# brown-ivl/manus

Hardware: AMD Instinct MI355X
Metric: train iters/sec (fwd+bwd) 300k Gaussians @1080p, 8 views; PSNR parity (higher is better)
Workload: dtype f32

## Files before the change

### manus_amd/csrc/raster_fwd.hip

```cpp
#include <atomic>
#include <mutex>

#include "instance_math.h"
#include "il_list.h"

#include <cstdlib>
#include <cstring>
#include <map>
#include <string>
#include <vector>

thread_local char g_mgr_err[512] = {0};

int g_mgr_prof_on = 0;
namespace {
struct ProfRec { const char* name; hipEvent_t a, b; };
std::vector<ProfRec> g_prof_recs;
std::vector<hipEvent_t> g_prof_pool;
hipEvent_t prof_event() {
    if (!g_prof_pool.empty()) { hipEvent_t e = g_prof_pool.back(); g_prof_pool.pop_back(); return e; }
    hipEvent_t e;
    if (hipEventCreate(&e) != hipSuccess) return nullptr;
    return e;
}
}

void mgr_prof_begin(const char* name, hipStream_t stream) {
    ProfRec r{name, prof_event(), prof_event()};
    if (r.a) (void)hipEventRecord(r.a, stream);
    g_prof_recs.push_back(r);
}
void mgr_prof_end(hipStream_t stream) {
    if (!g_prof_recs.empty() && g_prof_recs.back().b) (void)hipEventRecord(g_prof_recs.back().b, stream);
}

static std::string g_prof_filter;
static int g_prof_period = 1, g_prof_seen = 0;
bool mgr_prof_match(const char* name) {
    if (!(g_prof_filter.empty() || g_prof_filter == name)) return false;
    return g_prof_period <= 1 || (g_prof_seen++ % g_prof_period) == 0;
}
extern "C" int mgr_profile_sample_every(int n) {
    g_prof_period = n < 1 ? 1 : n;
    g_prof_seen = 0;
    return MGR_OK;
}

extern "C" int mgr_profile_enable(int on) {
    g_mgr_prof_on = on ? 1 : 0;
    return MGR_OK;
}

extern "C" int mgr_profile_filter(const char* kernel_name) {
    g_prof_filter = kernel_name ? kernel_name : "";
    return MGR_OK;
}

extern "C" int mgr_profile_report(char* buf, size_t len, void* stream_) {
    hipStream_t stream = (hipStream_t)stream_;
    MGR_HIP(hipStreamSynchronize(stream));
    std::map<std::string, std::pair<long, double>> agg;
    std::vector<std::string> order;
    for (auto& r : g_prof_recs) {
        float ms = 0.f;
        if (r.a && r.b && hipEventElapsedTime(&ms, r.a, r.b) == hipSuccess) {
            auto it = agg.find(r.name);
            if (it == agg.end()) { order.push_back(r.name); agg[r.name] = {1, ms}; }
            else { it->second.first += 1; it->second.second += ms; }
        }
        if (r.a) g_prof_pool.push_back(r.a);
        if (r.b) g_prof_pool.push_back(r.b);
    }
    g_prof_recs.clear();
    std::string out;
    for (auto& n : order) {
        char line[256];
        snprintf(line, sizeof(line), "%s %ld %.6f\n", n.c_str(), agg[n].first, agg[n].second);
        out += line;
    }
    if (buf && len) {
        size_t k = out.size() < len - 1 ? out.size() : len - 1;
        memcpy(buf, out.data(), k);
        buf[k] = 0;
    }
    return MGR_OK;
}

extern "C" int mgr_version(void) { return MGR_VERSION; }
int mgr_bwd_variant_bits(void);
extern "C" int mgr_raster_repair_max_tiles(void) { return MGR_REP_MAX_TILES; }

extern "C" int mgr_build_variant(void) {
    int bits = mgr_bwd_variant_bits();
#ifdef FWD_KO_DEEP
    bits |= 1;
#endif
#if defined(MGR_STATS) || defined(MGR_TIMELINE) || defined(FWD_PROF) || defined(BIN_PROF) || defined(DBS_PROF)
    bits |= 2;
#endif
#if defined(FWD_PF1) || defined(FWD_LDS_PIPE1)
    bits |= 4;
#endif
    if (MGR_BIN_BLOCK != 1024 || MGR_GREC_BYTES != 64 || MGR_DB_BUCKETS != 1024 || MGR_DB_ITEM != 768 || MGR_DB_RANK_MAX != 2048 ||
        MGR_DB_RANK_LARGE != 3072)
        bits |= 4;
    return bits;
}
extern "C" const char* mgr_last_error(void) { return g_mgr_err; }

extern "C" int mgr_raster_record_bytes(void) { return (int)sizeof(MgrGRec); }
extern "C" size_t mgr_raster_workspace_bytes(int V, int N, int W, int H, int64_t cap) {
    return mgr_layout(V, N, W, H, cap).total;
}

__device__ __forceinline__ uint32_t block_excl_scan(uint32_t val, uint32_t* s_wave ,
                                                    uint32_t& block_total) {
    const int lane = threadIdx.x & 63, wave = threadIdx.x >> 6, nw = blockDim.x >> 6;
    const uint32_t incl = mgr_wave_incl_scan_u32(val);
    if (lane == 63) s_wave[wave] = incl;
    __syncthreads();
    if (threadIdx.x == 0) {
        uint32_t run = 0;
        for (int w = 0; w < nw; ++w) {
            uint32_t t = s_wave[w];
            s_wave[w] = run;
            run += t;
        }
        s_wave[nw] = run;
    }
    __syncthreads();
    block_total = s_wave[nw];
    uint32_t r = s_wave[wave] + incl - val;
    __syncthreads();
    return r;
}

#ifndef MGR_FWD_GRID
#define MGR_FWD_GRID (256 * 24)
#endif
#ifndef PRE_THREADS
#define PRE_THREADS 512
#endif
#define EMIT_THREADS 1024

struct DbRange { float zmin, scale; };
__device__ __forceinline__ DbRange db_range_reduce(const uint32_t* __restrict__ slots , int nslots, uint32_t* s_zr ) {
    uint32_t lo_c = 0u, hi = 0u;
    for (int k = threadIdx.x; k < nslots; k += blockDim.x) { lo_c = max(lo_c, slots[2 * k]); hi = max(hi, slots[2 * k + 1]); }
    lo_c = mgr_wave_max_u32(lo_c); hi = mgr_wave_max_u32(hi);
    if ((threadIdx.x & 63) == 0 && hi) { atomicMax(&s_zr[0], lo_c); atomicMax(&s_zr[1], hi); }
    __syncthreads();
    lo_c = s_zr[0]; hi = s_zr[1];
    DbRange r;
    r.zmin = __uint_as_float(~lo_c);
    const float ext = __uint_as_float(hi) - r.zmin;
    r.scale = (hi != 0u && ext > 0.0f) ? (float)(MGR_DB_BUCKETS - 1) / ext : 0.0f;
    return r;
}
__device__ __forceinline__ uint32_t db_bucket(float z, const DbRange r) {
    const float f = (z - r.zmin) * r.scale;
    return f > 0.0f ? min((uint32_t)f, (uint32_t)MGR_DB_BUCKETS - 1u) : 0u;
}
__device__ __forceinline__ bool db_takes_part(int radius, ushort4 rc, unsigned long long am) {
    const uint32_t tiles = (uint32_t)((rc.z - rc.x) * (rc.w - rc.y));
    return radius > 0 && tiles > 0u && (tiles > 64u || am != 0ull);
}

__device__ __forceinline__ void pre_tail(int N, int gx, int gy, int v, int i, const ProjOut& po, float op_i,
                                         const float col[3], uint32_t* s_scan, uint32_t* s_hist, int lds_hist,
                                         MgrGRec* __restrict__ grec, float* __restrict__ depth,
                                         ushort4* __restrict__ rect, unsigned long long* __restrict__ alive,
                                         uint32_t* __restrict__ pair_off, uint32_t* __restrict__ tile_count,
                                         int32_t* __restrict__ radii, MgrHeader* hdr, uint32_t* __restrict__ zr_slot,
                                         const uint32_t* __restrict__ zcut_v = nullptr) {
    const int tid = threadIdx.x, T = gx * gy;
    const int radius = po.radius, x0 = po.x0, y0 = po.y0, x1 = po.x1, y1 = po.y1;
    const uint32_t tiles = (uint32_t)((x1 - x0) * (y1 - y0));
    {
        const uint32_t zb = (radius > 0 && tiles > 0u) ? __float_as_uint(po.zv) : 0u;
        const uint32_t wmax = mgr_wave_max_u32(zb), wminc = mgr_wave_max_u32(zb ? ~zb : 0u);
        if ((tid & 63) == 0 && wmax) { atomicMax(&s_scan[23], wmax); atomicMax(&s_scan[22], wminc); }
    }
    unsigned long long amask = ~0ull;
    if (radius > 0 && !(zcut_v && tiles <= 64)) {
        const bool small = tiles <= 64;
        const MgrCull cull = mgr_cull_init(po.px, po.py, po.ca, po.cb, po.cc, mgr_qmax(op_i));
        if (small) amask = 0ull;
        int k = 0;
// ... 1310 lines not shown
        const uint4 q = db_rec[(size_t)v * N + p];
        r.gid = db_order[(size_t)v * N + p];
        const uint32_t w = q.y & 0xFFFFu, h = q.y >> 16;
        r.xy = ((uint32_t)((int)(q.x & 0xFFFFu) - (int)box.x) & 0xFFFFu) | ((uint32_t)((int)(q.x >> 16) - (int)box.y) << 16);
        r.wh = q.y;
        r.tiles = w * h;
        r.alo = q.z; r.ahi = q.w;
    }
    return r;
}
__device__ __noinline__ BinRec bin_spread_lane(uint32_t j, const BinRec cur, const uint32_t* s_vend) {
    BinRec r = {0u, 0u, 0u, 0u, 0u, 0u};
    const bool on = j < s_vend[63];
    int lo = 0, hi = 63;
    while (lo < hi) {
        const int mid = (lo + hi) >> 1;
        if (s_vend[mid] > j) hi = mid; else lo = mid + 1;
    }
    BinRec q;
    q.xy = (uint32_t)__shfl((int)cur.xy, lo, 64); q.wh = (uint32_t)__shfl((int)cur.wh, lo, 64);
    q.alo = (uint32_t)__shfl((int)cur.alo, lo, 64); q.ahi = (uint32_t)__shfl((int)cur.ahi, lo, 64);
    q.gid = (uint32_t)__shfl((int)cur.gid, lo, 64); q.tiles = (uint32_t)__shfl((int)cur.tiles, lo, 64);
    if (!on) return r;
    if (q.tiles <= 64u) return q;
    const uint32_t piece = j - (lo ? s_vend[lo - 1] : 0u), qw = q.wh & 0xFFFFu, per_row = (qw + 63u) / 64u;
    const uint32_t row = piece / per_row, px = piece - row * per_row, ww = min(64u, qw - 64u * px);
    r.xy = ((uint32_t)(bin_x0(q.xy) + (int)(64u * px)) & 0xFFFFu) | ((uint32_t)(bin_y0(q.xy) + (int)row) << 16);
    r.wh = ww | (1u << 16);
    const unsigned long long ones = ww >= 64u ? ~0ull : ((1ull << ww) - 1ull);
    r.alo = (uint32_t)ones; r.ahi = (uint32_t)(ones >> 32);
    r.gid = q.gid;
    r.tiles = ww;
    return r;
}

__device__ __forceinline__ void bin_batch_by_instance(const BinRec& r, const BinRec* s_rec, uint32_t* s_cur, int bw, int lane,
                                                      uint32_t* __restrict__ sorted_gid, uint32_t cap) {
    const int g = lane >> 4, kq = lane & 15;
    const unsigned long long quad_ok = __ballot(r.tiles <= 16u);
    int i = 0;
#pragma unroll 1
    while (i < 64) {
        if ((i & 3) == 0 && ((quad_ok >> i) & 0xFull) == 0xFull) {
            const BinRec q = s_rec[i + g];
            const uint32_t w = q.wh & 0xFFFFu;
            const uint32_t ty = (uint32_t)(((float)kq + 0.5f) * __frcp_rn((float)max(w, 1u)));
            const uint32_t tx = kq - ty * w;
            const unsigned long long am = ((unsigned long long)q.ahi << 32) | q.alo;
            const bool valid = (uint32_t)kq < q.tiles && ((am >> kq) & 1ull);
            uint32_t* cur = &s_cur[valid ? (bin_y0(q.xy) + (int)ty) * bw + bin_x0(q.xy) + (int)tx : 0];
            uint32_t pa = 0, pb = 0, pc = 0, pd = 0;
            if (valid && g == 0) pa = atomicAdd(cur, 1u);
            __builtin_amdgcn_wave_barrier();
            if (valid && g == 1) pb = atomicAdd(cur, 1u);
            __builtin_amdgcn_wave_barrier();
            if (valid && g == 2) pc = atomicAdd(cur, 1u);
            __builtin_amdgcn_wave_barrier();
            if (valid && g == 3) pd = atomicAdd(cur, 1u);
            __builtin_amdgcn_wave_barrier();
            const uint32_t pos = pa | pb | pc | pd;
            if (valid && pos < cap) sorted_gid[pos] = q.gid;
            i += 4;
        } else {
            const BinRec q = s_rec[i];
            if (q.tiles) {
                const uint32_t w = q.wh & 0xFFFFu;
                const unsigned long long am = ((unsigned long long)q.ahi << 32) | q.alo;
                const bool small = q.tiles <= 64u;
                for (uint32_t k = (uint32_t)lane; k < q.tiles; k += 64) {
                    const uint32_t ty = k / w, tx = k - ty * w;
                    if (small && !((am >> k) & 1ull)) continue;
                    const uint32_t pos = atomicAdd(&s_cur[(bin_y0(q.xy) + (int)ty) * bw + bin_x0(q.xy) + (int)tx], 1u);
                    if (pos < cap) sorted_gid[pos] = q.gid;
                }
            }
            __builtin_amdgcn_wave_barrier();
            i += 1;
        }
    }
}

#define BIN_PAIR_CAP 1024
#ifdef BIN_PROF
__device__ unsigned long long g_binprof[8 * 4096];
#define BP(k) { const long long now_ = wall_clock64(); acc_[k] += now_ - tp_; tp_ = now_; }
#else
#define BP(k)
#endif
#define BIN_SC_THREADS 192
__constant__ unsigned long long c_row_comb[65] = {0x0000000000000000ull, 0x5555555555555555ull, 0x1111111111111111ull, 0x1041041041041041ull, 0x0101010101010101ull, 0x1004010040100401ull, 0x1001001001001001ull, 0x0100040010004001ull, 0x0001000100010001ull, 0x0040001000040001ull, 0x1000010000100001ull, 0x0000100000400001ull, 0x0001000001000001ull, 0x0010000004000001ull, 0x0100000010000001ull, 0x1000000040000001ull, 0x0000000100000001ull, 0x0000000400000001ull, 0x0000001000000001ull, 0x0000004000000001ull, 0x0000010000000001ull, 0x0000040000000001ull, 0x0000100000000001ull, 0x0000400000000001ull, 0x0001000000000001ull, 0x0004000000000001ull, 0x0010000000000001ull, 0x0040000000000001ull, 0x0100000000000001ull, 0x0400000000000001ull, 0x1000000000000001ull, 0x4000000000000001ull, 0x0000000000000001ull, 0x0000000000000001ull, 0x0000000000000001ull, 0x0000000000000001ull, 0x0000000000000001ull, 0x0000000000000001ull, 0x0000000000000001ull, 0x0000000000000001ull, 0x0000000000000001ull, 0x0000000000000001ull, 0x0000000000000001ull, 0x0000000000000001ull, 0x0000000000000001ull, 0x0000000000000001ull, 0x0000000000000001ull, 0x0000000000000001ull, 0x0000000000000001ull, 0x0000000000000001ull, 0x0000000000000001ull, 0x0000000000000001ull, 0x0000000000000001ull, 0x0000000000000001ull, 0x0000000000000001ull, 0x0000000000000001ull, 0x0000000000000001ull, 0x0000000000000001ull, 0x0000000000000001ull, 0x0000000000000001ull, 0x0000000000000001ull, 0x0000000000000001ull, 0x0000000000000001ull, 0x0000000000000001ull, 0x0000000000000001ull};
#define BIN_SC_FIXED_BYTES (2 * 64 * sizeof(BinRec) + 2 * BIN_PAIR_CAP * 4 + 3 * 64 * 4 + 16 + 66 * 8)
#define BIN_MID_TILES 1536
__device__ __forceinline__ bool bin_sc_mine(ushort4 box, int masks) {
    const uint32_t tb = (uint32_t)box.z * (uint32_t)box.w;
    if (tb == 0u) return false;
    const int tier = tb <= (uint32_t)BIN_MID_TILES ? BIN_MID_TILES : (tb <= (uint32_t)BIN_SMALL_TILES ? BIN_SMALL_TILES : 0);
    return tier == masks;
}
template <int MASKS, bool SPREAD>
__global__ __launch_bounds__(BIN_SC_THREADS) void k_bin_scatter(int N, int T, int nblk, int bb, const uint32_t* __restrict__ db_nvis,
                                                                const ushort4* __restrict__ db_bbox,
                                                                const uint32_t* __restrict__ db_order,
                                                                const uint4* __restrict__ db_rec,
                                                                const uint32_t* __restrict__ bin_mat,
                                                                uint32_t* __restrict__ sorted_gid, uint32_t cap,
                                                                MgrHeader* hdr, int skipped) {
    constexpr bool SMALL = MASKS > 0;
    extern __shared__ __attribute__((aligned(16))) uint32_t s_mem[];
    BinRec* s_rec = (BinRec*)s_mem;
    unsigned long long* s_mask = (unsigned long long*)(s_mem + 2 * 64 * (sizeof(BinRec) / 4));
    uint32_t* s_pairs = (uint32_t*)(s_mask + MASKS);
    uint32_t* s_gid = s_pairs + 2 * BIN_PAIR_CAP;
    uint32_t* s_info = s_gid + 2 * 64;
    unsigned long long* s_comb = (unsigned long long*)(s_info + 4);
    uint32_t* s_vend = (uint32_t*)(s_comb + 66);
    uint32_t* s_cur = s_vend + 64;
    const int v = blockIdx.y, b = blockIdx.x, tid = threadIdx.x, lane = tid & 63, wave = tid >> 6;
    const ushort4 box = db_bbox[v];
    if (!bin_sc_mine(box, MASKS)) {
        if (MASKS == BIN_MID_TILES && skipped && b == 0 && tid == 0) {
            const uint32_t tb = (uint32_t)box.z * (uint32_t)box.w;
            if ((tb > (uint32_t)BIN_SMALL_TILES && (skipped & MGR_SKIP_BOX_LARGE)) || (tb > (uint32_t)BIN_MID_TILES && tb <= (uint32_t)BIN_SMALL_TILES && (skipped & MGR_SKIP_BOX_MID)))
                atomicOr(&hdr->overflow, MGR_OVF_TIER);
        }
        return;
    }
    const uint32_t nvis = db_nvis[v], p0 = (uint32_t)b * (uint32_t)bb;
    if (p0 >= nvis) return;
    const uint32_t p1 = min(p0 + (uint32_t)bb, nvis);
    const int bw = box.z;
    const int nbatch = (int)((p1 - p0 + 63u) / 64u);
    BinRec nxt = {0u, 0u, 0u, 0u, 0u, 0u};
    if (wave == 0) nxt = bin_load(N, v, p0 + lane, nvis, box, db_order, db_rec);
    {
        const int TB = (int)box.z * (int)box.w;
        const uint32_t* row = bin_mat + ((size_t)v * nblk + b) * T;
        int k = tid;
        for (; k + 3 * BIN_SC_THREADS < TB; k += 4 * BIN_SC_THREADS) {
            const uint32_t a0 = row[k], a1 = row[k + BIN_SC_THREADS], a2 = row[k + 2 * BIN_SC_THREADS], a3 = row[k + 3 * BIN_SC_THREADS];
            s_cur[k] = a0; s_cur[k + BIN_SC_THREADS] = a1; s_cur[k + 2 * BIN_SC_THREADS] = a2; s_cur[k + 3 * BIN_SC_THREADS] = a3;
        }
        for (; k < TB; k += BIN_SC_THREADS) s_cur[k] = row[k];
        if (SMALL) for (k = tid; k < TB; k += BIN_SC_THREADS) s_mask[k] = 0ull;
        if (tid < 65) s_comb[tid] = c_row_comb[tid];
    }
    const unsigned long long lt = (1ull << lane) - 1ull;
#ifdef BIN_PROF
    long long acc_[6] = {0, 0, 0, 0, 0, 0};
    const long long t00_ = wall_clock64();
    long long tp_ = t00_;
#endif
    int src_it = 0;
    uint32_t v_total = 0, v_off = 0;
    bool v_mapped = false;
    BinRec cur = {0u, 0u, 0u, 0u, 0u, 0u};
    bool last_emitted = false;
    bool met_big = false;
#pragma unroll 1
    for (int it = 0; SPREAD || it <= nbatch; ++it) {
        __syncthreads();
        BP(5)
        if (wave == 0) {
            const int d = it & 1;
            if (SPREAD && last_emitted) break;
            if (SPREAD || it < nbatch) {
                BinRec r;
                if constexpr (!SPREAD) {
                    r = nxt;
                    BP(0)
                    if (it + 1 < nbatch) nxt = bin_load(N, v, p0 + 64u * (uint32_t)(it + 1) + lane, nvis, box, db_order, db_rec);
                } else {
                if (v_off >= v_total) {
                    cur = nxt;
                    BP(0)
                    ++src_it;
                    if (src_it < nbatch) nxt = bin_load(N, v, p0 + 64u * (uint32_t)src_it + lane, nvis, box, db_order, db_rec);
                    const uint32_t cw = cur.wh & 0xFFFFu, ch = cur.wh >> 16;
                    v_mapped = __ballot(cur.tiles > 64u) != 0ull;
                    v_off = 0u;
                    v_total = 64u;
                    if (v_mapped) {
                        met_big = true;
                        const uint32_t nl = cur.tiles == 0u ? 0u : (cur.tiles <= 64u ? 1u : ch * ((cw + 63u) / 64u));
                        const uint32_t ve = mgr_wave_incl_scan_u32(nl);
                        v_total = (uint32_t)__builtin_amdgcn_readlane((int)ve, 63);
                        s_vend[lane] = ve;
                        __builtin_amdgcn_wave_barrier();
                        if (v_total == 0u) v_total = 1u;
                    }
                }
                r = cur;
                if (v_mapped) r = bin_spread_lane(v_off + (uint32_t)lane, cur, s_vend);
                v_off += 64u;
                last_emitted = v_off >= v_total && src_it >= nbatch;
                }
                const unsigned long long am = ((unsigned long long)r.ahi << 32) | r.alo;
                const bool big = !SPREAD && r.tiles > 64u;
                const bool use = r.tiles != 0u && !big;
                const uint32_t w = r.wh & 0xFFFFu;
                unsigned long long amE = 0ull;
                if (use) {
                    const unsigned long long rb = w >= 64u ? ~0ull : ((1ull << w) - 1ull);
                    const unsigned long long evens = rb * s_comb[min(w, 64u)];
                    const unsigned long long rowm = (bin_y0(r.xy) & 1) ? (w >= 64u ? 0ull : evens << w) : evens;
                    amE = am & rowm;
                }
                const unsigned long long amU = use ? am : 0ull;
                const uint32_t cntE = (uint32_t)__popcll(amE), cntO = (uint32_t)__popcll(amU & ~amE);
                const uint32_t incl = mgr_wave_incl_scan_u32(cntE | (cntO << 16));
                const uint32_t P = (uint32_t)__builtin_amdgcn_readlane((int)incl, 63);
                const uint32_t PE = P & 0xFFFFu, PO = P >> 16;
                BP(1)
                const bool any_big = !SPREAD && __ballot(big) != 0ull;
                met_big = met_big || any_big;
                if (!any_big && PE + PO <= (uint32_t)BIN_PAIR_CAP) {
                    uint32_t* pl = s_pairs + d * BIN_PAIR_CAP;
                    uint32_t oE = (incl & 0xFFFFu) - cntE, oO = (incl >> 16) - cntO;
                    const float rw = __frcp_rn((float)max(w, 1u));
                    const int org = bin_y0(r.xy) * bw + bin_x0(r.xy);
                    unsigned long long m = amU;
                    while (m) {
                        const uint32_t k = (uint32_t)__builtin_ctzll(m);
                        m &= m - 1ull;
                        const uint32_t ty = (uint32_t)(((float)k + 0.5f) * rw), tx = k - ty * w;
                        const uint32_t isE = (uint32_t)((amE >> k) & 1ull);
                        const uint32_t at = isE ? oE : (uint32_t)BIN_PAIR_CAP - 1u - oO;
                        oE += isE;
                        oO += 1u - isE;
                        pl[at] = (uint32_t)(org + (int)ty * bw + (int)tx) | ((uint32_t)lane << 16);
                    }
                    s_gid[d * 64 + lane] = r.gid;
                    if (lane == 0) s_info[d] = P | (last_emitted ? 0x80000000u : 0u);
                } else {
                    s_rec[d * 64 + lane] = r;
                    if (lane == 0) s_info[d] = 0x7FFFFFFFu | (last_emitted ? 0x80000000u : 0u);
                }
                BP(2)
            }
        } else if (it >= 1) {
            const int d = (it - 1) & 1;
            const uint32_t Praw = s_info[d], Pboth = Praw & 0x7FFFFFFFu;
            if (Pboth != 0x7FFFFFFFu) {
                const bool odd = wave == 2;
                const uint32_t P = odd ? Pboth >> 16 : Pboth & 0xFFFFu;
                const uint32_t* const plist = s_pairs + d * BIN_PAIR_CAP;
                auto pl = [&](uint32_t i) -> uint32_t { return plist[odd ? (uint32_t)BIN_PAIR_CAP - 1u - i : i]; };
                const uint32_t* gl = s_gid + d * 64;
                uint32_t pr_n = lane < P ? pl((uint32_t)lane) : 0u;
                if (SMALL) {
                    uint32_t first_p = 0u, rank_p = 0u, gid_p = 0u, src_p = 0u;
                    bool valid_p = false;
#pragma unroll 1
                    for (uint32_t c = 0; c < P + 64; c += 64) {
                        const bool valid = c + lane < P;
                        const uint32_t pr = pr_n;
                        if (c + 64 < P) pr_n = (c + 64 + lane < P) ? pl(c + 64u + (uint32_t)lane) : 0u;
                        const uint32_t t = pr & 0xFFFFu;
                        if (valid) atomicOr(&s_mask[t], 1ull << lane);
                        __builtin_amdgcn_wave_barrier();
                        const unsigned long long mm = valid ? *(volatile unsigned long long*)&s_mask[t] : (1ull << lane);
                        const uint32_t rank = (uint32_t)__popcll(mm & lt);
                        const bool leader = valid && rank == 0u;
                        uint32_t first = 0u;
                        if (leader) {
                            first = atomicAdd(&s_cur[t], (uint32_t)__popcll(mm));
                            s_mask[t] = 0ull;
                        }
                        const uint32_t gid = gl[pr >> 16];
                        if (c > 0) {
                            const uint32_t f = (uint32_t)__shfl((int)first_p, (int)src_p, 64);
                            const uint32_t pos = f + rank_p;
                            if (valid_p && pos < cap) sorted_gid[pos] = gid_p;
                        }
                        first_p = first; rank_p = rank; gid_p = gid; valid_p = valid;
                        src_p = (uint32_t)__builtin_ctzll(mm);
                    }
                } else {
#pragma unroll 1
                    for (uint32_t c = 0; c < P; c += 64) {
                        const bool valid = c + lane < P;
                        const uint32_t pr = pr_n;
                        if (c + 64 < P) pr_n = (c + 64 + lane < P) ? pl(c + 64u + (uint32_t)lane) : 0u;
                        const uint32_t t = pr & 0xFFFFu;
                        uint32_t pos = 0u, cend = 1u;
                        if (valid) {
                            pos = atomicAdd(&s_cur[t], 1u);
                            cend = *(volatile uint32_t*)&s_cur[t];
                        }
                        const uint32_t gid = gl[pr >> 16];
                        unsigned long long todo = __ballot(valid && cend - pos > 1u);
                        while (todo) {
                            const int first = __builtin_ctzll(todo);
                            const uint32_t tstar = (uint32_t)__builtin_amdgcn_readlane((int)t, first);
                            const bool in = valid && t == tstar;
                            const unsigned long long grp = __ballot(in);
                            if (in) pos = cend - (uint32_t)__popcll(grp) + (uint32_t)__popcll(grp & lt);
                            todo &= ~grp;
                        }
                        if (valid && pos < cap) sorted_gid[pos] = gid;
                    }
                }
                BP(3)
            } else if (wave == 1) {
                const BinRec r = s_rec[d * 64 + lane];
                bin_batch_by_instance(r, s_rec + d * 64, s_cur, bw, lane, sorted_gid, cap);
                BP(4)
            }
            if (Praw & 0x80000000u) break;
        }
    }
    if (wave == 0 && lane == 0 && met_big && (*(volatile uint32_t*)&hdr->tiers & 4u) == 0u) atomicOr(&hdr->tiers, 4u);
#ifdef BIN_PROF
    {
        const int wid = blockIdx.y * gridDim.x + blockIdx.x;
        if (lane == 0 && wid < 4096) {
            if (wave == 0) { g_binprof[wid * 8 + 0] = acc_[0]; g_binprof[wid * 8 + 1] = acc_[1]; g_binprof[wid * 8 + 2] = acc_[2];
                             g_binprof[wid * 8 + 5] = (unsigned long long)(tp_ - t00_); g_binprof[wid * 8 + 6] = (unsigned long long)t00_;
                             g_binprof[wid * 8 + 7] = (unsigned long long)tp_; }
            else { g_binprof[wid * 8 + 3] = acc_[3]; g_binprof[wid * 8 + 4] = acc_[4]; }
        }
    }
#endif
}

struct FwdRec {
    float4 a, b;
    float c;
};

#ifdef MGR_STATS
__device__ unsigned long long g_fhist[5][65];
extern "C" int mgr_debug_fhist(unsigned long long* dst) {
    return (int)hipMemcpyFromSymbol(dst, HIP_SYMBOL(g_fhist), sizeof(unsigned long long) * 5 * 65);
}
#define FH(r, c, v) do { const int c_ = (c); const unsigned long long v_ = (unsigned long long)(v); if (lane == 0) atomicAdd(&g_fhist[r][c_], v_); } while (0)
#endif


#ifdef FWD_PROF
__device__ unsigned long long g_fprof[8];
extern "C" int mgr_debug_fprof(unsigned long long* dst) {
    return (int)hipMemcpyFromSymbol(dst, HIP_SYMBOL(g_fprof), sizeof(unsigned long long) * 8);
}
#ifndef FWD_PROF_MIN
#define FWD_PROF_MIN 0u
#endif
#ifndef FWD_PROF_MAX
#define FWD_PROF_MAX 0xFFFFFFFFu
#endif
#define FP(k) { const long long now_ = wall_clock64(); if (fp_on_) facc_[k] += now_ - ftp_; ftp_ = now_; }
#else
#define FP(k)
#endif
#ifndef FWD_WAVES_EU
#define FWD_WAVES_EU 4
#endif
#define FWD_OCC __attribute__((amdgpu_waves_per_eu(FWD_WAVES_EU, FWD_WAVES_EU)))
#ifdef MGR_TIMELINE
#define TLW_PER_WAVE 24
__device__ unsigned long long g_tlw[MGR_FWD_GRID * 4 * TLW_PER_WAVE * 4];
extern "C" int mgr_debug_timeline_w(void* dst, unsigned int* n) {
    *n = MGR_FWD_GRID * 4 * TLW_PER_WAVE;
    hipError_t e = hipMemcpyFromSymbol(dst, HIP_SYMBOL(g_tlw), sizeof(g_tlw));
    return (int)e;
}
#endif
__device__ __forceinline__ float mgr_sel(unsigned long long m, float a, float b) {
    float r;
    asm("v_cndmask_b32 %0, %1, %2, %3" : "=v"(r) : "v"(b), "v"(a), "s"(m));
    return r;
}
__device__ __forceinline__ uint32_t mgr_selu(unsigned long long m, uint32_t a, uint32_t b) {
    uint32_t r;
    asm("v_cndmask_b32 %0, %1, %2, %3" : "=v"(r) : "v"(b), "v"(a), "s"(m));
    return r;
}
__device__ __forceinline__ bool mgr_fwd_pair_step(const float4& R0, const float4& R1, const float4& R2, const float4& R3, const float4& R4,
                                                  const mgr_v2f fpx2, const mgr_v2f fpy2, float& Tr, mgr_v2f& C01, float& C2, uint32_t& last,
                                                  unsigned long long& done_m, const unsigned long long exec_m) {
    mgr_v2f al;
    unsigned long long ma, mb;
    mgr_pair_alpha_masks(R0, R1, R2, fpx2, fpy2, al, ma, mb);
    {
        const unsigned long long keep = ma & ~done_m;
        const float a = mgr_sel(keep, al.x, 0.0f);
        const float testT = Tr * (1.0f - a);
        const unsigned long long stop = __builtin_amdgcn_ballot_w64(testT < 0.0001f);
        const unsigned long long contrib = keep & ~stop;
        const float w = mgr_sel(contrib, a * Tr, 0.0f);
        C01 += mgr_v2f{R3.x, R3.y} * w;
        C2 += R4.x * w;
        Tr = mgr_sel(stop, Tr, testT);
        last = mgr_selu(contrib, __float_as_uint(R4.z), last);
        done_m |= stop;
    }
    {
        const unsigned long long keep = mb & ~done_m;
        const float a = mgr_sel(keep, al.y, 0.0f);
        const float testT = Tr * (1.0f - a);
        const unsigned long long stop = __builtin_amdgcn_ballot_w64(testT < 0.0001f);
        const unsigned long long contrib = keep & ~stop;
        const float w = mgr_sel(contrib, a * Tr, 0.0f);
// ... 1002 lines not shown
        MGR_HIP(side.init());
        MGR_HIP(hipEventRecord(side.fork, stream));
        MGR_HIP(hipStreamWaitEvent(side.stream, side.fork, 0));
        { MGR_PROF("k_tile_split", stream); hipLaunchKernelGGL(k_tile_split, dim3(256), dim3(SORT_THREADS), 0, stream,
                           tile_start, (const uint32_t*)(ws + L.tile_queue), (unsigned long long*)(ws + L.keys),
                           (unsigned long long*)(ws + L.keys2), (uint4*)(ws + L.groups),
                           (uint32_t*)(ws + L.sorted_gid), hdr, (uint32_t)cap); }
        { MGR_PROF("k_tile_sort_small", side.stream); hipLaunchKernelGGL(k_tile_sort_small, dim3(256 * 8), dim3(256), 0, side.stream,
                           tile_start, (const uint32_t*)(ws + L.tile_queue),
                           (const unsigned long long*)(ws + L.keys), (uint32_t*)(ws + L.sorted_gid), hdr,
                           (uint32_t)cap); }
        MGR_HIP(hipEventRecord(side.join, side.stream));
        { MGR_PROF("k_tile_sort", stream); hipLaunchKernelGGL(k_tile_sort, dim3(512), dim3(RS_THREADS), SORT_LDS_KEYS * 8 + RS_WAVES * 256 * 4 + 256, stream,
                           tile_start, (const uint32_t*)(ws + L.tile_queue),
                           (const unsigned long long*)(ws + L.keys), (const unsigned long long*)(ws + L.keys2),
                           (const uint4*)(ws + L.groups), (uint32_t*)(ws + L.sorted_gid), hdr, (uint32_t)cap); }
        MGR_HIP(hipStreamWaitEvent(stream, side.join, 0));
        MGR_LAUNCH_CHECK("k_tile_sort", stream, debug);
    }
    }
    if (!do_blend) return MGR_OK;
    { MGR_PROF("k_blend_fwd", stream); hipLaunchKernelGGL(k_blend_fwd, dim3(MGR_FWD_GRID), dim3(256), 0, stream, N, W, H, gx, gy, VT, bg,
                       (const uint32_t*)(ws + L.tile_queue), (const uint4*)(ws + L.tile_qrec), (const uint32_t*)(ws + L.sorted_gid), (const MgrGRec*)(ws + L.grec), out_color,
                       (uint32_t*)(ws + L.n_contrib), (uint32_t*)(ws + L.tile_done), (uint32_t*)(ws + L.tile_qdone),
                       (float4*)(ws + L.ckpt), hdr, (const uint32_t*)(ws + L.tile_zused), (uint32_t*)(ws + L.tile_qend), bg_filled ? 1 : 0); }
    if (repair && N > 0) {
        { MGR_PROF("k_repair_scan", stream);
          hipLaunchKernelGGL(k_repair_prep, dim3(V), dim3(256), 0, stream, T, gx, hdr, rep_all, (const uint32_t*)(ws + L.tile_zused),
                             (const uint32_t*)(ws + L.tile_zwin));
          hipLaunchKernelGGL(k_repair_scan, dim3(REP_SCAN_SEGS, V), dim3(REP_SCAN_THREADS), 0, stream, N, T, gx, hdr, rep_all, (const int32_t*)radii,
                             (const ushort4*)(ws + L.rect), (const float*)(ws + L.depth), (const MgrGRec*)(ws + L.grec)); }
        { MGR_PROF("k_repair_blend", stream);
          hipLaunchKernelGGL(k_repair_blend, dim3(128), dim3(RS_THREADS), REP_BLEND_LDS, stream, N, W, H, gx, T, hdr, rep_all, bg,
                             (uint32_t*)(ws + L.sorted_gid), (const MgrGRec*)(ws + L.grec), out_color, (uint32_t*)(ws + L.n_contrib),
                             (uint32_t*)(ws + L.tile_qdone), (float4*)(ws + L.ckpt)); }
        MGR_LAUNCH_CHECK("k_repair_blend", stream, debug);
    }
    IlListArgs ll = g_loss_list.take(workspace);
    if (ll.nbx) {
        if (ll.H != H || ll.W != W || ll.list_views != V) return mgr_fail(MGR_EINVAL, "attached loss list: views or image size differ from the forward's");
        ll.tile_start = tile_start;
    }
    const int n_item_blocks = (VT + 255) / 256;
    const MgrFeatStamp stamp = {{(uint32_t)V, (uint32_t)N, (uint32_t)W, (uint32_t)H, (uint32_t)cap}, use_cut ? MGR_FEAT_CUT : 0u};
    { MGR_PROF("k_fwd_items", stream); hipLaunchKernelGGL(k_fwd_items, dim3((unsigned)(n_item_blocks + ll.nbx * V)), dim3(256), 0, stream, (const uint4*)(ws + L.tile_qrec),
                       (const uint32_t*)(ws + L.tile_qdone), (uint32_t*)(ws + L.tile_done), (uint4*)(ws + L.items), hdr,
                       N, T, (const uint32_t*)(ws + L.sorted_gid), (const float*)(ws + L.depth), (const uint32_t*)(ws + L.tile_zused),
                       (const uint32_t*)(ws + L.tile_qend), (uint32_t*)(ws + L.tile_zcut), g_mirror.take(workspace),
                       g_cut_frac, (uint32_t)g_cut_min, g_cut_range, g_cut_rel, gx, g_cut_interior,
                       (const uint32_t*)(ws + L.tile_queue), VT, (unsigned char*)(ws + L.tile_bgok), (const float*)out_color, bg, rep_all,
                       (uint32_t)g_cut_penalty, (uint32_t*)(ws + L.tile_zwin), ll, n_item_blocks, stamp); }
    MGR_LAUNCH_CHECK("k_blend_fwd", stream, debug);
    return MGR_OK;
}

extern "C" int mgr_raster_forward(int V, int N, int W, int H, const float* cams, const float* bg,
                                  const float* means3D, int64_t s_means, const float* cov3D,
                                  int64_t s_cov, const float* colors, int64_t s_col,
                                  const float* opacity, int64_t s_op, float* out_color,
                                  int32_t* radii, void* workspace, size_t workspace_bytes,
                                  int64_t cap, int flags, void* stream_) {
    return raster_forward_impl(V, N, W, H, cams, bg, means3D, s_means, cov3D, s_cov, colors, s_col, opacity, s_op,
                               nullptr, out_color, radii, workspace, workspace_bytes, cap, flags, stream_);
}

extern "C" int mgr_views_forward(int V, int N, int B, int n_articulated, int sh_half, int W, int H, const float* cams, const float* bg,
                                 const float* xyz, const float* log_scale, const float* rot,
                                 const float* opacity_logit, const float* f_dc, const float* f_rest,
                                 const float* skin_w, const float* transforms, float* out_color,
                                 int32_t* radii, void* workspace, size_t workspace_bytes, int64_t cap,
                                 int flags, void* stream_) {
    if (N > 0 && (!xyz || !log_scale || !rot || !opacity_logit || !f_dc || !f_rest || (skin_w && !transforms)))
        return mgr_fail(MGR_EINVAL, "mgr_views_forward: null pointer");
    if (skin_w && (B <= 0 || B > MGR_MAX_BONES)) return mgr_fail(MGR_EINVAL, "mgr_views_forward: bad B");
    if (skin_w && (n_articulated < 0 || n_articulated > N)) return mgr_fail(MGR_EINVAL, "mgr_views_forward: bad n_articulated");
    if (sh_half && ((uintptr_t)f_rest & 15)) return mgr_fail(MGR_EINVAL, "mgr_views_forward: fp16 f_rest must be 16-byte aligned");
    const CanonInputs ci = {B, skin_w ? n_articulated : 0, sh_half ? 1 : 0, xyz, log_scale, rot, opacity_logit, f_dc, f_rest, skin_w, transforms};
    return raster_forward_impl(V, N, W, H, cams, bg, nullptr, 0, nullptr, 0, nullptr, 0, nullptr, 0, &ci, out_color,
                               radii, workspace, workspace_bytes, cap, flags, stream_);
}

#ifdef BIN_PROF
extern "C" int mgr_binprof(unsigned long long* out) {
    MGR_HIP(hipMemcpyFromSymbol(out, HIP_SYMBOL(g_binprof), 8 * 8 * 4096));
    return 0;
}
#endif
extern "C" int mgr_raster_layout(int V, int N, int W, int H, int64_t cap, size_t* out, int n_out) {
    const MgrLayout L = mgr_layout(V, N, W, H, cap);
    const size_t v[] = {L.header, L.grec, L.depth, L.rect, L.alive, L.pair_off, L.tile_count, L.tile_start,
                        L.tile_cursor, L.tile_done, L.tile_queue, L.chunk_start, L.items, L.ckpt, L.keys,
                        L.sorted_gid, L.final_T, L.n_contrib, L.pair_tag, L.pair_grad, L.total, L.inst_grad, L.inst_tag,
                        L.db_nvis, L.db_bbox, L.db_order, L.tile_zcut, L.tile_zused, L.tile_qend, L.tile_rep, L.rep_unit, L.rep_cnt, L.tile_zwin};
    const int n = (int)(sizeof(v) / sizeof(v[0]));
    for (int i = 0; i < n && i < n_out; ++i) out[i] = v[i];
    return n;
}

__global__ void k_debug_pair_alpha(int n, const float* __restrict__ rec, const int32_t* __restrict__ px,
                                   const int32_t* __restrict__ py, float* __restrict__ alpha, int32_t* __restrict__ valid) {
    const int i = blockIdx.x * blockDim.x + threadIdx.x;
    if (i >= n) return;
    float pb[MGR_PAIR_FLOATS];
    const float* r = rec + (size_t)i * 6;
    mgr_pair_store(pb, 0, r[0], r[1], r[2], r[3], r[4], r[5], 0.f, 0.f, 0.f, 1u);
    mgr_pair_pad(pb);
    const float4 R0 = make_float4(pb[0], pb[1], pb[2], pb[3]), R1 = make_float4(pb[4], pb[5], pb[6], pb[7]),
                 R2 = make_float4(pb[8], pb[9], pb[10], pb[11]);
    const mgr_v2f fpx2 = {(float)px[i], (float)px[i]}, fpy2 = {(float)py[i], (float)py[i]};
    mgr_v2f dx, dy, G, al;
    bool va, vb;
    mgr_pair_alpha(R0, R1, R2, fpx2, fpy2, dx, dy, G, al, va, vb);
    alpha[i] = al.x;
    valid[i] = va ? 1 : 0;
}

extern "C" int mgr_debug_pair_alpha(int n, const float* rec, const int32_t* px, const int32_t* py, float* alpha,
                                    int32_t* valid, void* stream_) {
    if (n < 0 || (n > 0 && (!rec || !px || !py || !alpha || !valid))) return mgr_fail(MGR_EINVAL, "mgr_debug_pair_alpha: bad arguments");
    if (n == 0) return MGR_OK;
    hipStream_t stream = (hipStream_t)stream_;
    hipLaunchKernelGGL(k_debug_pair_alpha, dim3((n + 255) / 256), dim3(256), 0, stream, n, rec, px, py, alpha, valid);
    MGR_LAUNCH_CHECK("k_debug_pair_alpha", stream, 0);
    return MGR_OK;
}

static int mgr_overflow_code(uint32_t ovf) {
    if (ovf & MGR_OVF_PAIRS) return mgr_fail(MGR_EOVERFLOW, "pair capacity exceeded");
    if (ovf & MGR_OVF_CUT) return mgr_fail(MGR_ECUT, "depth cut violated: run the forward again without MGR_FWD_DEPTH_CUT");
    if (ovf & MGR_OVF_TIER) return mgr_fail(MGR_ETIER, "a skipped binning launch was needed: run the forward again without MGR_FWD_SKIP_*");
    return MGR_OK;
}

extern "C" int mgr_raster_status_sync(const void* workspace, int64_t* num_pairs, int32_t* overflow,
                                      void* stream_) {
    hipStream_t stream = (hipStream_t)stream_;
    uint32_t h[2] = {0, 0};
    MGR_HIP(hipMemcpyAsync(h, workspace, 8, hipMemcpyDeviceToHost, stream));
    MGR_HIP(hipStreamSynchronize(stream));
    if (num_pairs) *num_pairs = h[0];
    if (overflow) *overflow = (int32_t)h[1];
    return mgr_overflow_code(h[1]);
}

extern "C" int mgr_raster_status_tiers_sync(const void* workspace, int64_t* num_pairs, int32_t* overflow, int32_t* tiers,
                                            void* stream_) {
    hipStream_t stream = (hipStream_t)stream_;
    uint32_t h[64];
    static_assert(offsetof(MgrHeader, sort_near_large) / 4 < 64, "status words beyond the copied part of the header");
    MGR_HIP(hipMemcpyAsync(h, workspace, sizeof(h), hipMemcpyDeviceToHost, stream));
    MGR_HIP(hipStreamSynchronize(stream));
    if (num_pairs) *num_pairs = h[0];
    if (overflow) *overflow = (int32_t)h[1];
    if (tiers) {
        const uint32_t sb = h[offsetof(MgrHeader, sort_big) / 4], sn = h[offsetof(MgrHeader, sort_near_large) / 4], sl = h[offsetof(MgrHeader, sort_large) / 4];
        const uint32_t near_max = MGR_TIERS_NEAR_MASK, beyond_max = MGR_TIERS_BEYOND_SMALL_MASK;
        *tiers = (int32_t)(h[offsetof(MgrHeader, tiers) / 4] | ((sb < near_max ? sb : near_max) << MGR_TIERS_NEAR_SMALL_SHIFT) |
                           ((sn < near_max ? sn : near_max) << MGR_TIERS_NEAR_LARGE_SHIFT) | ((sl < beyond_max ? sl : beyond_max) << MGR_TIERS_BEYOND_SMALL_SHIFT));
    }
    return mgr_overflow_code(h[1]);
}

extern "C" int mgr_raster_debug_binning_sync(const void* workspace, int V, int N, int W, int H,
                                             int64_t cap, int view, int32_t* tile_ranges_host,
                                             int32_t* point_list_host, int64_t max_pairs,
                                             void* stream_) {
    hipStream_t stream = (hipStream_t)stream_;
// ... 24 lines not shown
```

Before: 782.5.

## Split bin-scatter pair-list production across two producer waves

```diff
diff --git a/manus_amd/csrc/raster_fwd.hip b/manus_amd/csrc/raster_fwd.hip
--- a/manus_amd/csrc/raster_fwd.hip
+++ b/manus_amd/csrc/raster_fwd.hip
@@ -104,6 +104,9 @@
     if (MGR_BIN_BLOCK != 1024 || MGR_GREC_BYTES != 64 || MGR_DB_BUCKETS != 1024 || MGR_DB_ITEM != 768 || MGR_DB_RANK_MAX != 2048 ||
         MGR_DB_RANK_LARGE != 3072)
         bits |= 4;
+#if defined(BIN_SC_PRODUCERS) && BIN_SC_PRODUCERS != 2
+    bits |= 4;
+#endif
     return bits;
 }
 extern "C" const char* mgr_last_error(void) { return g_mgr_err; }
@@ -1580,12 +1583,19 @@
 
 #define BIN_PAIR_CAP 1024
 #ifdef BIN_PROF
-__device__ unsigned long long g_binprof[8 * 4096];
+#define BINPROF_SLOTS 16
+__device__ unsigned long long g_binprof[BINPROF_SLOTS * 4096];
 #define BP(k) { const long long now_ = wall_clock64(); acc_[k] += now_ - tp_; tp_ = now_; }
 #else
 #define BP(k)
 #endif
-#define BIN_SC_THREADS 192
+#ifndef BIN_SC_PRODUCERS
+#define BIN_SC_PRODUCERS 2
+#endif
+#if BIN_SC_PRODUCERS != 1 && BIN_SC_PRODUCERS != 2
+#error "BIN_SC_PRODUCERS is 1 or 2"
+#endif
+#define BIN_SC_THREADS (BIN_SC_PRODUCERS == 2 ? 256 : 192)
 __constant__ unsigned long long c_row_comb[65] = {0x0000000000000000ull, 0x5555555555555555ull, 0x1111111111111111ull, 0x1041041041041041ull, 0x0101010101010101ull, 0x1004010040100401ull, 0x1001001001001001ull, 0x0100040010004001ull, 0x0001000100010001ull, 0x0040001000040001ull, 0x1000010000100001ull, 0x0000100000400001ull, 0x0001000001000001ull, 0x0010000004000001ull, 0x0100000010000001ull, 0x1000000040000001ull, 0x0000000100000001ull, 0x0000000400000001ull, 0x0000001000000001ull, 0x0000004000000001ull, 0x0000010000000001ull, 0x0000040000000001ull, 0x0000100000000001ull, 0x0000400000000001ull, 0x0001000000000001ull, 0x0004000000000001ull, 0x0010000000000001ull, 0x0040000000000001ull, 0x0100000000000001ull, 0x0400000000000001ull, 0x1000000000000001ull, 0x4000000000000001ull, 0x0000000000000001ull, 0x0000000000000001ull, 0x0000000000000001ull, 0x0000000000000001ull, 0x0000000000000001ull, 0x0000000000000001ull, 0x0000000000000001ull, 0x0000000000000001ull, 0x0000000000000001ull, 0x0000000000000001ull, 0x0000000000000001ull, 0x0000000000000001ull, 0x0000000000000001ull, 0x0000000000000001ull, 0x0000000000000001ull, 0x0000000000000001ull, 0x0000000000000001ull, 0x0000000000000001ull, 0x0000000000000001ull, 0x0000000000000001ull, 0x0000000000000001ull, 0x0000000000000001ull, 0x0000000000000001ull, 0x0000000000000001ull, 0x0000000000000001ull, 0x0000000000000001ull, 0x0000000000000001ull, 0x0000000000000001ull, 0x0000000000000001ull, 0x0000000000000001ull, 0x0000000000000001ull, 0x0000000000000001ull, 0x0000000000000001ull};
 #define BIN_SC_FIXED_BYTES (2 * 64 * sizeof(BinRec) + 2 * BIN_PAIR_CAP * 4 + 3 * 64 * 4 + 16 + 66 * 8)
 #define BIN_MID_TILES 1536
@@ -1628,8 +1638,11 @@
     const uint32_t p1 = min(p0 + (uint32_t)bb, nvis);
     const int bw = box.z;
     const int nbatch = (int)((p1 - p0 + 63u) / 64u);
+    constexpr bool TWO = BIN_SC_PRODUCERS == 2 && !SPREAD;
+    const bool prodO = TWO && wave == 3;
+    const bool prod = wave == 0 || prodO;
     BinRec nxt = {0u, 0u, 0u, 0u, 0u, 0u};
-    if (wave == 0) nxt = bin_load(N, v, p0 + lane, nvis, box, db_order, db_rec);
+    if (prod) nxt = bin_load(N, v, p0 + lane, nvis, box, db_order, db_rec);
     {
         const int TB = (int)box.z * (int)box.w;
         const uint32_t* row = bin_mat + ((size_t)v * nblk + b) * T;
@@ -1658,7 +1671,7 @@
     for (int it = 0; SPREAD || it <= nbatch; ++it) {
         __syncthreads();
         BP(5)
-        if (wave == 0) {
+        if (prod) {
             const int d = it & 1;
             if (SPREAD && last_emitted) break;
             if (SPREAD || it < nbatch) {
@@ -1716,6 +1729,18 @@
                     uint32_t oE = (incl & 0xFFFFu) - cntE, oO = (incl >> 16) - cntO;
                     const float rw = __frcp_rn((float)max(w, 1u));
                     const int org = bin_y0(r.xy) * bw + bin_x0(r.xy);
+                    if constexpr (TWO) {
+                        unsigned long long m = prodO ? amU & ~amE : amE;
+                        uint32_t at = prodO ? (uint32_t)BIN_PAIR_CAP - 1u - oO : oE;
+                        const uint32_t step = prodO ? ~0u : 1u;
+                        while (m) {
+                            const uint32_t k = (uint32_t)__builtin_ctzll(m);
+                            m &= m - 1ull;
+                            const uint32_t ty = (uint32_t)(((float)k + 0.5f) * rw), tx = k - ty * w;
+                            pl[at] = (uint32_t)(org + (int)ty * bw + (int)tx) | ((uint32_t)lane << 16);
+                            at += step;
+                        }
+                    } else {
                     unsigned long long m = amU;
                     while (m) {
                         const uint32_t k = (uint32_t)__builtin_ctzll(m);
@@ -1727,9 +1752,12 @@
                         oO += 1u - isE;
                         pl[at] = (uint32_t)(org + (int)ty * bw + (int)tx) | ((uint32_t)lane << 16);
                     }
-                    s_gid[d * 64 + lane] = r.gid;
-                    if (lane == 0) s_info[d] = P | (last_emitted ? 0x80000000u : 0u);
-                } else {
+                    }
+                    if (!prodO) {
+                        s_gid[d * 64 + lane] = r.gid;
+                        if (lane == 0) s_info[d] = P | (last_emitted ? 0x80000000u : 0u);
+                    }
+                } else if (!prodO) {
                     s_rec[d * 64 + lane] = r;
                     if (lane == 0) s_info[d] = 0x7FFFFFFFu | (last_emitted ? 0x80000000u : 0u);
                 }
@@ -1738,7 +1766,8 @@
         } else if (it >= 1) {
             const int d = (it - 1) & 1;
             const uint32_t Praw = s_info[d], Pboth = Praw & 0x7FFFFFFFu;
-            if (Pboth != 0x7FFFFFFFu) {
+            if (wave == 3) {
+            } else if (Pboth != 0x7FFFFFFFu) {
                 const bool odd = wave == 2;
                 const uint32_t P = odd ? Pboth >> 16 : Pboth & 0xFFFFu;
                 const uint32_t* const plist = s_pairs + d * BIN_PAIR_CAP;
@@ -1812,10 +1841,12 @@
     {
         const int wid = blockIdx.y * gridDim.x + blockIdx.x;
         if (lane == 0 && wid < 4096) {
-            if (wave == 0) { g_binprof[wid * 8 + 0] = acc_[0]; g_binprof[wid * 8 + 1] = acc_[1]; g_binprof[wid * 8 + 2] = acc_[2];
-                             g_binprof[wid * 8 + 5] = (unsigned long long)(tp_ - t00_); g_binprof[wid * 8 + 6] = (unsigned long long)t00_;
-                             g_binprof[wid * 8 + 7] = (unsigned long long)tp_; }
-            else { g_binprof[wid * 8 + 3] = acc_[3]; g_binprof[wid * 8 + 4] = acc_[4]; }
+            unsigned long long* o = g_binprof + (size_t)wid * BINPROF_SLOTS;
+            if (wave == 0) { o[0] = acc_[0]; o[1] = acc_[1]; o[2] = acc_[2]; o[5] = (unsigned long long)(tp_ - t00_);
+                             o[6] = (unsigned long long)t00_; o[7] = (unsigned long long)tp_; o[12] = acc_[5]; }
+            else if (wave == 1) { o[3] = acc_[3]; o[4] = acc_[4]; o[14] = acc_[5]; }
+            else if (wave == 2) { o[11] = acc_[3]; o[15] = acc_[5]; }
+            else { o[8] = acc_[0]; o[9] = acc_[1]; o[10] = acc_[2]; o[13] = acc_[5]; }
         }
     }
 #endif
@@ -2984,7 +3015,7 @@
 
 #ifdef BIN_PROF
 extern "C" int mgr_binprof(unsigned long long* out) {
-    MGR_HIP(hipMemcpyFromSymbol(out, HIP_SYMBOL(g_binprof), 8 * 8 * 4096));
+    MGR_HIP(hipMemcpyFromSymbol(out, HIP_SYMBOL(g_binprof), 8 * BINPROF_SLOTS * 4096));
     return 0;
 }
 #endif
```

Result: no change. 787.6 (median of 6 runs) (+0.7%).
